# jrl-umi3218/jrl-walkgen

Measured on AMD Instinct MI355X. Metric: QP-MPC ticks/sec (batch=4096, N=16), higher is better.
Workload: dtype f64

## Files before the change

### jrl-walkgen_amd/csrc/wg_ql_device.hpp

```cpp
#pragma once
#include <hip/hip_runtime.h>

#include <type_traits>

#include "wg_wave.hpp"
#include "wg_ql_view.hpp"
#include "wg_ql_phases.hpp"

namespace wg {

#define WG_BACKSUB(q, s, nact, lane)                                                                   \
  do {                                                                                                 \
    if constexpr (P::kNM > 0 && P::kNM + 12 <= 48) backsub_lds<48>(q, s, nact, lane, q.sc0);          \
    else if (P::kNM == 0 && (P::kWideN || q.n >= 48) && (nact) <= 60) backsub_lds<96>(q, s, nact, lane, q.sc0);     \
    else if (P::kNM == 0 && !P::kRowOps && q.n >= 24 && (nact) <= 36) backsub_lds<48>(q, s, nact, lane, q.sc0); \
    else backsub(q, s, nact, lane);                                                                    \
  } while (0)
#define WG_SWEEP(q, s, nu, nact, lane) \
  do { if (P::kNM > 0 || (!P::kRowOps && q.n <= 64)) sweep_flat<P::kFixedLdz>(q, s, nu, nact, lane PT_SW_ARG); else sweep<(P::kRowOps ? WG_ELEM_GRP : 8), P::kWideN>(q, s, nu, nact, lane); } while (0)

#define QL_SCAN_ACCEPT                                                                        \
  if (wak <= 0.0) continue;                                                                   \
  double sumx = -sum * wak;                                                                   \
  if (k + 1 <= me) sumx = fabs(sumx);                                                         \
// ... 200 lines not shown
        xmag = 0.0;
        vfact = 1.0;
        WG_WSYNC();
        PT(PS_RESET_BODY);
      } else {
        iflag = 2;
        WG_REP(11) {
        typename ActiveParamsOf<P>::type ap;
        if constexpr (P::kCompact) ap = prob.active_params(q, nact, lane);
        for (int i = lane; i < n; i += 64) {
          double acc = q.d[i];
          if constexpr (P::kCompact) acc = prob.gdot_acc(q, i, q.x, acc);
          else {
            WG_UNROLL
            for (int j = 0; j < n; ++j) acc += Gm(i, j) * q.x[j];
          }
          PT_VIA(PS_RESID_GX, q.ww[i], acc);
          if constexpr (P::kCompact) acc = prob.grad_minus_active(q, ap, nact, i, acc);
          else {
            WG_UNROLL
            for (int k = 0; k < nact; ++k) {
              int kk = q.iact[k];
              if (kk <= m) acc -= q.lam[k] * Am(kk - 1, i);
              else if (kk <= mn) { if (kk - m - 1 == i) acc -= q.lam[k]; }
              else { if (kk - mn - 1 == i) acc += q.lam[k]; }
            }
          }
          q.ww[i] = acc;
        }
        if constexpr (P::kCompact) { prob.row_residuals(q, q.sc0, lane); WG_WSYNC(); }
        for (int k = lane; k < nact; k += 64) {
          int kk = q.iact[k];
          double sk;
          if (kk <= m) {
            if constexpr (P::kCompact) sk = q.sc0[kk - 1];
            else {
              sk = q.b[kk - 1];
              WG_UNROLL
              for (int i = 0; i < n; ++i) sk -= q.x[i] * Am(kk - 1, i);
            }
          } else if (kk <= mn) { int k1 = kk - m - 1; sk = prob.xl(q, k1) - q.x[k1]; }
          else { int k1 = kk - mn - 1; sk = -prob.xu(q, k1) + q.x[k1]; }
          s[k] = sk;
        }
        WG_WSYNC();
        }
        PT(PS_RESID_GRAD);
      }
      if (nact > 0) {
        {
          double sum0 = 0.0, sum1 = 0.0;
          const int i0 = lane, i1 = lane + 64;
          for (int j = 0; j < nact; ++j) {
            if (i0 == j) s[j] = (s[j] - sum0) / Rp(j, j);
            if (i1 == j) s[j] = (s[j] - sum1) / Rp(j, j);
            WG_WSYNC();
            double sj = s[j];
            if (i0 > j && i0 < nact) sum0 += Rp(j, i0) * sj;
            if (i1 > j && i1 < nact) sum1 += Rp(j, i1) * sj;
          }
        }
        PT(PS_RESID_FWD);
        if (P::kWideN || (P::kNM == 0 && n > 64 && n <= 128)) {
          double r0, r1;
          z_rows_times<(P::kRowOps ? WG_ELEM_GRP : 8)>(q, s, 0, nact, lane, r0, r1);
          q.x[lane] += r0; q.sc0[lane] = r0;
          if (lane + 64 < n) { q.x[lane + 64] += r1; q.sc0[lane + 64] = r1; }
        } else
        for (int i = lane; i < n; i += 64) {
          double sum = 0.0;
          WG_UNROLL
          for (int j = 0; j < nact; ++j) sum += s[j] * Zm(i, j);
          q.x[i] += sum;
          q.sc0[i] = sum;
        }
        WG_WSYNC();
        for (int j = lane; j < n; j += 64) {
          double acc = q.ww[j];
          if constexpr (P::kCompact) acc = prob.gdot_acc(q, j, q.sc0, acc);
          else {
            WG_UNROLL
            for (int i = 0; i < n; ++i) acc += q.sc0[i] * Gm(i, j);
          }
          q.ww[j] = acc;
        }
        WG_WSYNC();
      }
      PT(PS_RESID);
      zt_times_ww<P::kNM, (P::kRowOps ? WG_ELEM_GRP : 8), P::kWideN>(q, s, lane);
      PT(PS_ZTWW_RESID);
      if (nact != n) {
        if (P::kWideN || (P::kNM == 0 && n > 64 && n <= 128)) {
          double r0, r1;
          z_rows_times<(P::kRowOps ? WG_ELEM_GRP : 8)>(q, s, nact, n, lane, r0, r1);
          q.x[lane] -= r0;
          if (lane + 64 < n) q.x[lane + 64] -= r1;
        } else
        for (int i = lane; i < n; i += 64) {
          double sum = 0.0;
          WG_UNROLL
          for (int j = nact; j < n; ++j) sum += Zm(i, j) * s[j];
          q.x[i] -= sum;
        }
        info = 0;
        WG_WSYNC();
      }
      PT(PS_XSHIFT);
      if (nact != 0) {
        WG_BACKSUB(q, s, nact, lane);
        for (int k = lane; k < nact; k += 64) q.lam[k] += q.ww[k];
        WG_WSYNC();
      }
      PT(PS_BACKSUB_RESID);
      { double sm = 0.0; WG_REP(6) { sm = uni(xmag_sum(q, prob, vfact, lane)); WG_SINK(sm); } xmag = maxd(xmag, sm); }
      PT(PS_XMAG_RESID);
      if (iflag == itref) { st = ST_RESID; continue; }
      int kd = 0x7fffffff;
      for (int k = lane; k < nact; k += 64)
        if (!(q.lam[k] >= 0.0) && q.iact[k] > me) { kd = k < kd ? k : kd; }
      kd = uni(wave_min_int(kd));
      if (kd != 0x7fffffff) {
        LOG_EVENT(-q.iact[kd]);
        nact = drop_constraint(q, kd, nact, nact, lane);
        st = ST_RESID;
        continue;
      }
      if constexpr (kNan) x_suspect = x_suspect || x_has_non_numbers();
      st = ST_SCAN;
    }

    if (st == ST_SCAN) {
      next_scan: asm volatile("" : "+v"(lane));
      double bestv = 0.0, bestres = 0.0, bestw = 0.0;
      int bidx = -1;
      if (kNan && x_suspect) {
        if constexpr (kNan) {
          double cv = 0.0;
          int kn = knext;
          scan_nan_exact(q, prob, onha, cv, res, wsel, kn, lane);
          knext = uni(kn);
          bestv = uni(cv); bidx = -1;
        }
      } else
      WG_REP(1) {
      bestv = 0.0; bestres = 0.0; bestw = 0.0; bidx = -1;
      if constexpr (P::kCompact) {
        constexpr int NH = sizeof(prob.ax) / sizeof(double);
        double xs[2 * NH];
#pragma unroll
        for (int c = 0; c < 2 * NH; ++c) xs[c] = q.x[c];
        const bool has_foot = lane < 5 * prob.ns;
        const int kf = has_foot ? 1 + 4 * NH + lane : 0;
        const double wakf = q.wa[kf], bkf = q.b[kf];
        {
          const int k = lane + 1;
          const double wak = q.wa[k], bk = prob.bcop;
          double sum = -bk, asum = fabs(bk);
          prob.cop_row_dot(xs, sum, asum);
          if (prob.fj >= 0) {
            double t = q.x[2 * NH + prob.fj] * prob.fa(); sum += t; asum += fabs(t);
            t = q.x[2 * NH + prob.ns + prob.fj] * prob.fb(); sum += t; asum += fabs(t);
          }
          const double sumx = -sum * wak;
          {
            const double tempa = asum + fabs(sum);
            const double temp2 = asum + onha * fabs(sum);
            const bool take = (wak > 0.0) & !(sumx <= 0.0) & !(tempa <= asum) & !(temp2 <= tempa);
            bestv = take ? sumx : bestv; bestres = take ? sum : bestres; bestw = take ? wak : bestw; bidx = take ? k + 1 : bidx;
          }
        }
        {
          const int k = kf;
          const double wak = wakf, bk = bkf;
          double sum = -bk, asum = fabs(bk);
          const auto fr = prob.foot_row();
#pragma unroll
          for (int e = 0; e < 4; ++e) { const double t = q.x[fr.c[e]] * fr.v[e]; sum += t; asum += fabs(t); }
          const double sumx = -sum * wak;
          const double tempa = asum + fabs(sum);
          const double temp2 = asum + onha * fabs(sum);
          const bool take = has_foot & (wak > 0.0) & !(sumx <= 0.0) & !((bidx >= 0) & (sumx <= bestv)) & !(tempa <= asum) & !(temp2 <= tempa);
          bestv = take ? sumx : bestv; bestres = take ? sum : bestres; bestw = take ? wak : bestw; bidx = take ? k + 1 : bidx;
        }
      } else {
      if constexpr (P::kRowOps) {
        constexpr int kScanPasses = 3;
        double wak_p[kScanPasses], bk_p[kScanPasses], ra_p[kScanPasses], rb_p[kScanPasses];
        int rk_p[kScanPasses];
#pragma unroll
        for (int pp = 0; pp < kScanPasses; ++pp) {
          const int k = 1 + 64 * pp + lane;
          const bool in = k < m;
          const int kc = in ? k : 0;
          wak_p[pp] = in ? q.wa[kc] : 0.0; bk_p[pp] = q.b[kc];
          ra_p[pp] = prob.rowA[kc]; rb_p[pp] = prob.rowB[kc]; rk_p[pp] = prob.rowK[kc];
        }
#pragma unroll
        for (int pp = 0; pp < kScanPasses; ++pp) {
          const int k0 = 1 + 64 * pp;
          if (k0 >= m) break;
          const int k = k0 + lane;
          const int kc = k < m ? k : 0;
          const double wak = wak_p[pp], bk = bk_p[pp];
          double sum = -bk, temp = fabs(bk);
          prob.row_dot_both(q, kc, k0, ra_p[pp], rb_p[pp], rk_p[pp], q.x, sum, temp);
          QL_SCAN_ACCEPT;
        }
      } else if constexpr (HasRegRows<P>::value) {
        constexpr int NMr = P::kNM;
        const int ka = lane, kb = lane + 64;
        const bool ina = ka < m, inb = kb < m;
        const int mc = m > 0 ? m - 1 : 0;
        const int kca = ina ? ka : mc, kcb = inb ? kb : mc;
        const double waka = ina ? q.wa[kca] : 0.0, bka = q.b[kca], wakb = inb ? q.wa[kcb] : 0.0, bkb = q.b[kcb];
        double suma = -bka, tempa_ = fabs(bka), sumb = -bkb, tempb_ = fabs(bkb);
#pragma unroll
        for (int i0 = 0; i0 < NMr; i0 += 8) {
          double xs[8];
#pragma unroll
          for (int e = 0; e < 8; ++e) xs[e] = q.x[(i0 + e < n) ? i0 + e : n - 1];
#pragma unroll
          for (int e = 0; e < 8; ++e)
            if (i0 + e < NMr && i0 + e < n) {
              const double ta = xs[e] * prob.ar0[i0 + e]; suma += ta; tempa_ += fabs(ta);
              const double tb = xs[e] * prob.ar1[i0 + e]; sumb += tb; tempb_ += fabs(tb);
            }
        }
#pragma unroll
        for (int pp = 0; pp < 2; ++pp) {
          const int k = pp == 0 ? ka : kb;
          const double wak = pp == 0 ? waka : wakb, sum = pp == 0 ? suma : sumb;
          double temp = pp == 0 ? tempa_ : tempb_;
          QL_SCAN_ACCEPT;
        }
      } else
      for (int k0 = 0; k0 < m; k0 += 64) {
        const int k = k0 + lane;
        const bool in = k < m;
        const int kc = in ? k : m - 1;
        const double wak = in ? q.wa[kc] : 0.0, bk = q.b[kc];
        double sum = -bk, temp = fabs(bk);
        {
          constexpr int kG = 8;
          double ua[kG], ub[kG];
          auto fetch = [&](double (&u)[kG], int i) {
#pragma unroll
            for (int e = 0; e < kG; ++e) u[e] = Am(kc, i + e < n ? i + e : n - 1);
          };
          auto add = [&](const double (&u)[kG], int i) {
            double xs[kG];
#pragma unroll
            for (int e = 0; e < kG; ++e) xs[e] = q.x[i + e];
#pragma unroll
            for (int e = 0; e < kG; ++e) { const double t = xs[e] * u[e]; sum += t; temp += fabs(t); }
          };
          int i = 0;
          const int whole = n / kG * kG;
          if (whole > 0) {
            fetch(ua, 0);
            for (;;) {
              fetch(ub, i + kG);
              add(ua, i); i += kG;
              if (i >= whole) break;
              fetch(ua, i + kG);
              add(ub, i); i += kG;
              if (i >= whole) { 
#pragma unroll
                for (int e = 0; e < kG; ++e) ub[e] = ua[e];
                break;
              }
            }
#pragma unroll
            for (int e = 0; e < kG - 1; ++e)
              if (i + e < n) { const double t = q.x[i + e] * ub[e]; sum += t; temp += fabs(t); }
          } else {
            for (; i < n; ++i) { const double t = q.x[i] * Am(kc, i); sum += t; temp += fabs(t); }
          }
        }
        QL_SCAN_ACCEPT;
      }
      }
      if constexpr (P::kNM > 0) {
        const bool in = lane < n;
        const int kc = in ? lane : n - 1;
        const double w = q.wa[m + kc], xk = q.x[kc];
        const double s1 = prob.xl(q, kc) - xk;
        const bool upper = s1 < 0.0;
        const double sum = upper ? xk - prob.xu(q, kc) : s1;
        const bool take = in && !(w <= 0.0) && !(s1 == 0.0) && !(sum <= 0.0) && !(bidx >= 0 && sum <= bestv);
        bestv = take ? sum : bestv; bestres = take ? -sum : bestres; bestw = take ? w : bestw; bidx = take ? (upper ? kc + 1 + mn : kc + 1 + m) : bidx;
      } else
      for (int k = lane; k < n; k += 64) {
        const double w = q.wa[m + k];
        if (w <= 0.0) continue;
        bool lower = true;
        double sum = prob.xl(q, k) - q.x[k];
        if (sum == 0.0) continue;
        if (sum < 0.0) { sum = q.x[k] - prob.xu(q, k); lower = false; }
        if (sum <= 0.0) continue;
        if (bidx >= 0 && sum <= bestv) continue;
        bestv = sum; bestres = -sum; bestw = w; bidx = lower ? k + 1 + m : k + 1 + mn;
      }
      {
        int key = bidx < 0 ? -1 : (bidx > mn ? bidx - n : bidx);
        double v = bestv;
        int kk = key;
        wave_argmax_first(v, kk);
        kk = uni(kk);
        if (kk < 0) { bestv = 0.0; bidx = -1; }
        else {
          int src = -1;
          unsigned long long mask = __ballot(key == kk);
          src = __ffsll((long long)mask) - 1;
          bestv = rl(bestv, src);
          bestres = rl(bestres, src);
          bestw = rl(bestw, src);
          bidx = __builtin_amdgcn_readlane(bidx, src);
        }
      }
      WG_SINK(bestv); WG_SINK(bestres); WG_SINK(bestw); WG_SINK(bidx);
      }
      double cvmax = bestv;
      if (bidx >= 0) { res = bestres; knext = bidx; wsel = bestw; }
      PT(PS_SCAN);
      info = 0;
      if (WG_UBOOL(cvmax <= wg_kconst(vsmall))) { st = ST_CONVERGED; continue; }

      ++jfinc;
      if (jfinc == 0 || jfinc == ifinc) {
        if (jfinc == ifinc) {
          for (int i = lane; i < n; i += 64) {
            double sum = 2.0 * q.d[i];
            double sumx = fabs(sum);
            WG_UNROLL
            for (int j = 0; j < n; ++j) {
              double temp = Gm(i, j) * (q.wx[j] + q.x[j]);
              sum += temp;
              sumx += fabs(temp);
            }
            double dx = q.x[i] - q.wx[i];
            q.sc0[i] = sum * dx;
            q.sc1[i] = sumx * fabs(dx);
          }
          WG_WSYNC();
          double fdiff = 0.0, fdiffa = 0.0;
          WG_UNROLL
          for (int i = 0; i < n; ++i) { fdiff += q.sc0[i]; fdiffa += q.sc1[i]; }
          info = 2;
          double sum = fdiffa + fdiff;
          if (WG_UBOOL(sum <= fdiffa)) { st = ST_CONVERGED; continue; }
          double temp = fdiffa + onha * fdiff;
          if (WG_UBOOL(temp <= sum)) { st = ST_CONVERGED; continue; }
          jfinc = 0;
          info = 0;
        }
        for (int i = lane; i < n; i += 64) q.wx[i] = q.x[i];
        WG_WSYNC();
      }
      PT(PS_FDIFF);
      ++iterc;
      if (iterc > maxit) { info = 1; st = ST_FINISH; continue; }

      s = q.R + nact * (nact + 1) / 2;
      WG_REP(2)
      if (knext <= m) {
        if constexpr (P::kCompact) prob.fill_row(q, knext - 1, q.ww, lane);
        else if constexpr (HasRegRows<P>::value) prob.row_to(q, knext - 1, q.ww, lane);
        else for (int i = lane; i < n; i += 64) q.ww[i] = Am(knext - 1, i);
        WG_WSYNC();
        if constexpr (P::kCompact) prob.zt_row(q, s, knext - 1, lane);
        else if constexpr (P::kWideN && P::kRowOps) {
          constexpr int kNHc = P::kHorizon;
          const int k = knext - 1;
          const bool cop = k >= 1 && k <= 4 * kNHc;
          const int rr = cop ? ((k - 1) >> 2) : -1;
          const int si = cop ? prob.stepidx[rr] : 1;
          zt_times_ww_cop_tiled<kNHc>(q, s, lane, rr, !cop || (si >= 1 && si <= prob.ns));
        }
        else zt_times_ww<P::kNM, (P::kRowOps ? WG_ELEM_GRP : 8), P::kWideN>(q, s, lane);
      } else {
        int k1 = knext - m;
        double sg = 1.0;
        if (k1 > n) { k1 = knext - mn; sg = -1.0; }
        for (int i = lane; i < n; i += 64) {
          q.ww[i] = (i == k1 - 1) ? sg : 0.0;
          double z = Zm(k1 - 1, i);
          s[i] = (sg > 0.0) ? z : -z;
        }
        WG_WSYNC();
      }
      PT(PS_NEWNORMAL);
      double parnew = 0.0, parinc = 0.0, step = 0.0, sumy;
      int kdrop = -1;
      int route;
      if (nact == n) route = 1;
      else {
        WG_SWEEP(q, s, n, nact, lane);
        PT(PS_SWEEP);
        if (nact == 0) route = 0;
        else {
          double suma = 0.0, sumb = 0.0, sumc = 0.0;
          WG_REP(5) {
          if constexpr (P::kNM > 0) {
            constexpr int NM = P::kNM;
            if (lane < NM) {
              const bool in = lane < n;
              const double zi = in ? Zm(lane, nact) : 0.0, wi = in ? q.ww[lane] : 0.0;
              q.sc0[lane] = wi * zi; q.sc1[lane] = fabs(wi * zi); q.sc2[lane] = zi * zi;
            }
            WG_WSYNC();
            typedef __attribute__((address_space(3))) double lds_f64;
            const lds_f64 *src = (const lds_f64 *)(q.sc0 + (lane < 3 ? lane : 0) * (int)(q.sc1 - q.sc0));
            asm volatile("" : "+v"(src));
            double acc = 0.0;
#pragma unroll
            for (int i0 = 0; i0 < NM; i0 += kOsChunk) {
              double t[kOsChunk];
#pragma unroll
              for (int i = 0; i < kOsChunk; ++i) if (i0 + i < NM) t[i] = src[i0 + i];
#pragma unroll
              for (int i = 0; i < kOsChunk; ++i) if (i0 + i < NM) acc += t[i];
            }
            suma = rl(acc, 0); sumb = rl(acc, 1); sumc = rl(acc, 2);
            WG_WSYNC();
          } else {
            for (int i = lane; i < n; i += 64) {
              const double zi = Zm(i, nact), wi = q.ww[i];
              q.sc0[i] = wi * zi; q.sc1[i] = fabs(wi * zi); q.sc2[i] = zi * zi;
            }
            WG_WSYNC();
            const double *src = q.sc0 + (lane < 3 ? lane : 0) * (int)(q.sc1 - q.sc0);
            double acc = 0.0;
            int i = 0;
            for (; i + 8 <= n; i += 8) {
              double t[8];
#pragma unroll
              for (int e = 0; e < 8; ++e) t[e] = src[i + e];
#pragma unroll
              for (int e = 0; e < 8; ++e) acc += t[e];
            }
            for (; i < n; ++i) acc += src[i];
            suma = rl(acc, 0); sumb = rl(acc, 1); sumc = rl(acc, 2);
            WG_WSYNC();
          }
          WG_SINK(suma); WG_SINK(sumb); WG_SINK(sumc);
          }
          if (WG_UBOOL(!significant(sumb, fabs(suma)) || !(sumb > wg_kconst(vsmall)))) route = 1;
          else {
            sumc = sqrt(sumc);
            if (knext <= m) sumc /= wsel;
            if (WG_UBOOL(significant(sumc, fabs(suma)))) route = 0;
            else {
              PT_COUNT(PS_N_COORD);
              WG_BACKSUB(q, s, nact, lane);
              route = independent_coordinate(q, prob, knext, nact, vsmall, lane) ? 0 : 2;
            }
          }
        }
      }
      route = uni(route);
      PT(PS_ROUTE);
      PT_COUNT(PS_N_ROUTE);
      if (route != 0) PT_COUNT(PS_N_DEPENDENT);
      if (route != 0) {
        if (route == 1) WG_BACKSUB(q, s, nact, lane);
        kdrop = pick_drop<(P::kNM > 0), kNan>(q, nact, res, ratio, lane);
        info = -knext;
        if (kdrop < 0) { st = ST_CONVERGED; continue; }
        parinc = ratio;
        parnew = parinc;
      }

      bool dual_only = (route != 0);
      for (;;) {
        if (!dual_only) {
          sumy = s[nact];
          step = -res / sumy;
          parinc = step / sumy;
          kdrop = -1;
          if (nact > 0) {
            PT(PS_STEP_PRE);
            WG_REP(4) WG_BACKSUB(q, s, nact, lane);
            PT(PS_BACKSUB_STEP);
            WG_REP(7) { kdrop = pick_drop<(P::kNM > 0), kNan>(q, nact, res, ratio, lane); WG_SINK(kdrop); WG_SINK(ratio); }
            PT(PS_PICKDROP);
            if (kdrop >= 0) {
              double temp = 1.0 - ratio / parinc;
              if (WG_UBOOL(temp <= 0.0)) kdrop = -1;
              else { step = ratio * sumy; parinc = ratio; res = temp * res; }
            }
          }
          if constexpr (P::kNM > 0) {
            const int il = lane < n ? lane : n - 1;
            q.x[il] = q.x[il] + step * Zm(il, nact);
          } else
          for (int i = lane; i < n; i += 64) q.x[i] += step * Zm(i, nact);
          parnew += parinc;
          if constexpr (kNan) x_suspect = x_suspect || WG_UBOOL(!wg_sane(step) || !wg_sane(parinc));
          WG_WSYNC();
          if (nact < 1) break;
        }
        dual_only = false;
        if constexpr (P::kNM > 0) {
          if (nact > 0) {
            const int kl = lane < nact ? lane : nact - 1;
            const double l0 = q.lam[kl] - parinc * q.ww[kl];
            const int ia = q.iact[kl];
            q.lam[kl] = (ia > me) ? maxd(0.0, l0) : l0;
          }
        } else
        for (int k = lane; k < nact; k += 64) {
          double l = q.lam[k] - parinc * q.ww[k];
          if (q.iact[k] > me) l = maxd(0.0, l);
          q.lam[k] = l;
        }
        WG_WSYNC();
        if (kdrop < 0) break;
        {
          int nu = nact + 1;
          LOG_EVENT(-q.iact[kdrop]);
          nact = drop_constraint(q, kdrop, nu, nact, lane);
          double *snew = s - (nact + 1);
          if (nu > n) nu = n;
          for (int i0 = 0; i0 < nu; i0 += 64) {
            int i = i0 + lane;
            double v = (i < nu) ? s[i] : 0.0;
            WG_WSYNC();
            if (i < nu) snew[i] = v;
            WG_WSYNC();
          }
          s = snew;
          WG_SWEEP(q, s, nu, nact, lane);
        }
      }

      PT(PS_STEP);
      ql_activate(q, nact, knext, parnew, wsel, lane, n, mn);
      nact++;
      LOG_EVENT(knext);
      WG_WSYNC();
      PT(PS_ADD);
      double sm = 0.0;
      WG_REP(6) { sm = uni(xmag_sum(q, prob, vfact, lane)); WG_SINK(sm); }
      xmag = maxd(xmag, sm);
      PT(PS_XMAG_ADD);
      if (WG_UBOOL(sm < wg_kconst(xmagr) * xmag)) st = ST_RESET;
      else if (itref <= 0) st = ST_SCAN;
      else st = ST_RESID;
      if (q.nact_cap > 0 && nact > q.nact_cap) { cap_hit = true; break; }
      if (st == ST_SCAN) goto next_scan;
      continue;
    }

    if (st == ST_CONVERGED) {
      ++itref;
      jfinc = -1;
      if (itref == 1) { st = ST_RESID; continue; }
      st = ST_FINISH;
    }
  }
#undef LOG_EVENT
// ... 20 lines not shown
```

### jrl-walkgen_amd/csrc/wg_ql_herdt.hpp

```cpp
#pragma once
#include "wg_ql_device.hpp"

namespace wg {

constexpr int kSMaxQ = 4;
constexpr int kGvLd = 4;
constexpr int kQbLd = 32;

template <int NH, int NS>
__device__ __forceinline__ bool herdt_border_rows(const QlView &q, const double *gd, const double *Gv, double vsmall, int lane) {
  constexpr int M2 = 2 * NH;
  const int i = lane;
  const bool jerk = i < NH, foot = i >= NH && i < NH + NS, row = jerk || foot;
  const int fi = i - NH;
  const int gi = jerk ? i : M2 + (foot ? fi : 0);
  double acc[NS];
#pragma unroll
  for (int f = 0; f < NS; ++f)
    acc[f] = (jerk || (foot && f >= fi)) ? ((foot && f == fi) ? gd[gi] : Gv[gi * kGvLd + f]) : 0.0;
  const double dreg = jerk ? Rf(i, i) : 1.0;
  const int colbase = jerk ? i * (i + 1) / 2 : 0;
  const int khi = jerk ? i : 0;
  double rnext = (0 < khi) ? q.Rf[colbase] : 0.0;
  for (int k = 0; k < NH; ++k) {
// ... 363 lines not shown
    }
    const int cc = row - 2 * NH;
#pragma unroll
    for (int k0 = 0; k0 < 2 * NH; k0 += 8) {
      double gg[8], vv[8];
#pragma unroll
      for (int c = 0; c < 8; ++c) { gg[c] = Gv[(k0 + c) * kGvLd + cc]; vv[c] = v[k0 + c]; }
#pragma unroll
      for (int c = 0; c < 8; ++c) acc += gg[c] * vv[c];
    }
    for (int c = 0; c < n - 2 * NH; ++c) {
      const double g = (c == cc) ? gd[row] : Gv[row * kGvLd + c];
      acc += g * v[2 * NH + c];
    }
    return acc;
  }

  struct ActiveParams { double pa, pb, plam; int pr, ptype, pidx; };
  __device__ __forceinline__ ActiveParams active_params(const QlView &q, int nact, int lane) const {
    const int m = q.m, mn = q.mn;
    ActiveParams P;
    P.pa = 0.0; P.pb = 0.0; P.plam = 0.0; P.pr = -1; P.ptype = 4; P.pidx = -1;
    int rk = 0;
    if (lane < nact) {
      const int kk = q.iact[lane];
      P.plam = q.lam[lane];
      if (kk <= m) {
        rk = kk - 1;
        P.ptype = (rk >= 1 && rk <= 4 * NH) ? 0 : 1;
        if (rk == 0) P.ptype = 4;
      } else if (kk <= mn) { P.ptype = 2; P.pidx = kk - m - 1; }
      else { P.ptype = 3; P.pidx = kk - mn - 1; }
    }
    double *t = q.sc0;
    t[lane + 1] = ra;
    if (lane < 5 * ns) t[1 + 4 * NH + lane] = ga;
    WG_WSYNC();
    if (P.ptype <= 1) P.pa = t[rk];
    WG_WSYNC();
    t[lane + 1] = rb;
    if (lane < 5 * ns) t[1 + 4 * NH + lane] = gb;
    WG_WSYNC();
    if (P.ptype <= 1) P.pb = t[rk];
    WG_WSYNC();
    int *tk = reinterpret_cast<int *>(q.sc0);
    if (lane < 5 * ns) tk[lane] = gk;
    WG_WSYNC();
    if (P.ptype == 0) P.pr = (rk - 1) >> 2;
    else if (P.ptype == 1) P.pr = tk[rk - 1 - 4 * NH];
    WG_WSYNC();
    return P;
  }
  __device__ __forceinline__ double grad_minus_active(const QlView &q, const ActiveParams &P, int nact, int i, double acc) const {
    const bool xb = i < NH, jerk = i < 2 * NH;
    const int c = xb ? i : i - NH;
    int fjx = -1, fjy = -1;
    if (!jerk) { const int j = i - 2 * NH; if (j < ns) fjx = j; else fjy = j - ns; }
    for (int k = 0; k < nact; ++k) {
      const int type = __builtin_amdgcn_readlane(P.ptype, k);
      const double lam = rl(P.plam, k);
      if (type <= 1) {
        const double a = rl(P.pa, k), b = rl(P.pb, k);
        const int r = __builtin_amdgcn_readlane(P.pr, k);
        double e = 0.0;
        if (type == 0) {
          if (jerk) {
            const double ab = xb ? a : b;
            const int rc = (c <= r) ? r - c : 0;
            const double uu = u[rc];
            e = (c <= r) ? 0.0 + (0.0 + ab * uu) * -1.0 : 0.0;
          } else {
            const int sidx = stepidx[r];
            if (fjx >= 0) { const double v = (sidx == fjx + 1) ? 1.0 : 0.0; e = 0.0 + (0.0 + a * v) * 1.0; }
            else { const double v = (sidx == fjy + 1) ? 1.0 : 0.0; e = 0.0 + (0.0 + b * v) * 1.0; }
          }
        } else if (!jerk && r >= 0) {
          if (fjx >= 0) e = 0.0 + (0.0 + a * V_f[r * kSMaxQ + fjx]) * -1.0;
          else e = 0.0 + (0.0 + b * V_f[r * kSMaxQ + fjy]) * -1.0;
        }
        acc -= lam * e;
      } else if (type == 2) {
        if (__builtin_amdgcn_readlane(P.pidx, k) == i) acc -= lam;
      } else if (type == 3) {
        if (__builtin_amdgcn_readlane(P.pidx, k) == i) acc += lam;
      }
    }
    return acc;
  }
  __device__ __forceinline__ void row_residuals(const QlView &q, double *out, int lane) const {
    double xs[2 * NH];
#pragma unroll
    for (int c = 0; c < 2 * NH; ++c) xs[c] = q.x[c];
    {
      const int rk = lane + 1;
      double sk = q.b[rk];
#pragma unroll
      for (int c = 0; c < NH; ++c) sk -= xs[c] * ax[c];
#pragma unroll
      for (int c = 0; c < NH; ++c) sk -= xs[NH + c] * ay[c];
      if (fj >= 0) { sk -= q.x[2 * NH + fj] * fa(); sk -= q.x[2 * NH + ns + fj] * fb(); }
      out[rk] = sk;
    }
    if (lane < 5 * ns) {
      const int rk = 1 + 4 * NH + lane;
      double sk = q.b[rk];
      const FootRow fr = foot_row();
#pragma unroll
      for (int e = 0; e < 4; ++e) sk -= q.x[fr.c[e]] * fr.v[e];
      out[rk] = sk;
    }
    if (lane == 0) out[0] = q.b[0];
  }

  __device__ __forceinline__ double diag_check(const QlView &q, double vsmall, int lane) const {
    const int n = q.n;
    double dl = diag_b;
    for (int i = lane; i < n; i += 64) {
      const double wdi = q.wd[i];
      if (i >= 2 * NH) dl = maxd(dl, vsmall - wdi);
      const int j0 = (i + 1 > 2 * NH) ? i + 1 : 2 * NH;
      for (int j = j0; j < n; ++j) {
        const double gjj = q.wd[j], gij = G(q, i, j);
        double ga = -mind(wdi, gjj);
        const double gb = fabs(wdi - gjj) + fabs(gij);
        if (gb > 0.0) ga += gij * gij / gb;
        dl = maxd(dl, ga);
      }
    }
    return wave_max(dl);
  }

  __device__ __forceinline__ bool factor(const QlView &q, double vsmall, int lane) const {
    const int n = q.n;
    constexpr int M2 = 2 * NH;
    PT_LOCAL_BEGIN
    herdt_constant_blocks<NH>(q, R2, Z2, z2sign, lane);
    WG_WSYNC();
    const int nb = n - M2;
    PT_LOCAL(PS_CHOL);
    bool ok = true;
    if (nb == 2) ok = herdt_border_rows<NH, 1>(q, gd, Gv, vsmall, lane);
    else if (nb == 4) ok = herdt_border_rows<NH, 2>(q, gd, Gv, vsmall, lane);
    if (!WG_UBOOL(ok)) return false;
    WG_WSYNC();
    PT_LOCAL(PS_BORDER_ROWS);
    if (nb == 2) herdt_border_z<NH, 1>(q, lane);
    else if (nb == 4) herdt_border_z<NH, 2>(q, lane);
    WG_WSYNC();
    return true;
  }

  __device__ __forceinline__ void zt_row(const QlView &q, double *s, int rk, int lane) const {
    const int n = q.n;
    if (lane < n) {
      const int i = lane;
      const double *zc = q.Z + i * q.ldz;
      double acc = 0.0;
      if (rk >= 1 && rk <= 4 * NH) {
        constexpr int kZtChunk = 8;
        const int r = (rk - 1) >> 2;
#pragma unroll
        for (int j0 = 0; j0 < 2 * NH; j0 += kZtChunk) {
          if ((j0 < NH ? j0 : j0 - NH) > r) continue;
          double zz[kZtChunk], wv[kZtChunk];
#pragma unroll
          for (int c = 0; c < kZtChunk; ++c) { zz[c] = zc[j0 + c]; wv[c] = q.ww[j0 + c]; }
#pragma unroll
          for (int c = 0; c < kZtChunk; ++c) acc += zz[c] * wv[c];
        }
      }
      for (int j = 2 * NH; j < n; ++j) acc += zc[j] * q.ww[j];
      s[i] = acc;
    }
    WG_WSYNC();
  }
};

constexpr int kGvLdElem = kSMaxQ;
template <int NHC>
struct HerdtElemProbT {
  static constexpr bool kCompact = false;
  static constexpr bool kNanExact = WG_TICK_NAN_EXACT != 0;
  static constexpr bool kHasFactor = true;
  static constexpr bool kRowOps = true;
  static constexpr int kNM = 0;
  static constexpr bool kWideN = NHC >= 32;
  static constexpr int kFixedLdz = 0;
  static constexpr int kHorizon = NHC;
  struct NConst { static constexpr int v = NHC; __device__ __forceinline__ NConst &operator=(int) { return *this; } __device__ __forceinline__ operator int() const { return v; } };
  typename std::conditional<(NHC > 0), NConst, int>::type N;
  int ns;
  const double *Qb;
  const double *u;
  double *Gv;
  double *gd;
  const double *rowA, *rowB;
  const int *rowK, *stepidx;
  const double *V_f;
  const double *R2, *Z2;
  const unsigned long long *z2sign;
  int blocks_ok;
  __device__ __forceinline__ bool factor(const QlView &q, double vsmall, int lane) const {
    if ((int)N != 32 || ns < 1 || ns > 4) return false;
    constexpr int NHc = 32;
    herdt_constant_blocks<NHc>(q, R2, Z2, z2sign, lane);
    WG_WSYNC();
    bool ok = true;
    switch (ns) {
      case 1: ok = herdt_border_rows<NHc, 1>(q, gd, Gv, vsmall, lane); break;
      case 2: ok = herdt_border_rows<NHc, 2>(q, gd, Gv, vsmall, lane); break;
      case 3: ok = herdt_border_rows<NHc, 3>(q, gd, Gv, vsmall, lane); break;
      default: ok = herdt_border_rows<NHc, 4>(q, gd, Gv, vsmall, lane); break;
    }
    if (!WG_UBOOL(ok)) return false;
    WG_WSYNC();
    switch (ns) {
      case 1: herdt_border_z<NHc, 1>(q, lane); break;
      case 2: herdt_border_z<NHc, 2>(q, lane); break;
      case 3: herdt_border_z<NHc, 3>(q, lane); break;
      default: herdt_border_z<NHc, 4>(q, lane); break;
    }
    WG_WSYNC();
    return true;
  }
  __device__ __forceinline__ double G(const QlView &q, int i, int j) const {
    if (i == j) return gd[i];
    if (j < i) { const int t = i; i = j; j = t; }
    if (j < 2 * N) {
      if (i < N && j < N) return Qb[i * kQbLd + j];
      if (i >= N && j >= N) return Qb[(i - N) * kQbLd + (j - N)];
      return 0.0;
    }
    const int c = j - 2 * N;
    const bool xcol = c < ns, xrow = (i < N) || (i >= 2 * N && i < 2 * N + ns);
    if (xcol != xrow) return 0.0;
    return Gv[i * kGvLdElem + (xcol ? c : c - ns)];
  }
  __device__ __forceinline__ double Gd(const QlView &, int i) const { return gd[i]; }
  __device__ __forceinline__ void setGd(const QlView &, int i, double v) const { gd[i] = v; }
  __device__ __forceinline__ double xl(const QlView &, int) const { return -1e8; }
  __device__ __forceinline__ double xu(const QlView &, int) const { return 1e8; }
  __device__ __forceinline__ double A(const QlView &, int k, int i) const {
    if (k == 0) return 0.0;
    const double a = rowA[k], b = rowB[k];
    const int kk = rowK[k];
    if (k <= 4 * N) {
      const int r = kk;
      if (i < N) return (i <= r) ? 0.0 + (0.0 + a * u[r - i]) * -1.0 : 0.0;
      if (i < 2 * N) { const int c = i - N; return (c <= r) ? 0.0 + (0.0 + b * u[r - c]) * -1.0 : 0.0; }
      int j = i - 2 * N;
      if (j < ns) { const double v = (stepidx[r] == j + 1) ? 1.0 : 0.0; return 0.0 + (0.0 + a * v) * 1.0; }
      j -= ns;
      { const double v = (stepidx[r] == j + 1) ? 1.0 : 0.0; return 0.0 + (0.0 + b * v) * 1.0; }
    }
    if (kk < 0 || i < 2 * N) return 0.0;
    int j = i - 2 * N;
    if (j < ns) return 0.0 + (0.0 + a * V_f[kk * kSMaxQ + j]) * -1.0;
    j -= ns;
    return 0.0 + (0.0 + b * V_f[kk * kSMaxQ + j]) * -1.0;
  }
  template <bool ABS>
  __device__ __forceinline__ double row_dot(const QlView &, int k, const double *v, double acc) const {
    if (k == 0) return acc;
    const double a = rowA[k], b = rowB[k];
    const int kk = rowK[k];
    if (k <= 4 * N) {
      const int r = kk;
      for (int c = 0; c <= r; ++c) { const double t = v[c] * (0.0 + (0.0 + a * u[r - c]) * -1.0); acc += ABS ? fabs(t) : t; }
      for (int c = 0; c <= r; ++c) { const double t = v[N + c] * (0.0 + (0.0 + b * u[r - c]) * -1.0); acc += ABS ? fabs(t) : t; }
      const int j = stepidx[r] - 1;
      if (j >= 0 && j < ns) {
        { const double t = v[2 * N + j] * (0.0 + (0.0 + a * 1.0) * 1.0); acc += ABS ? fabs(t) : t; }
        { const double t = v[2 * N + ns + j] * (0.0 + (0.0 + b * 1.0) * 1.0); acc += ABS ? fabs(t) : t; }
      }
      return acc;
    }
    if (kk < 0) return acc;
    for (int j = 0; j < ns; ++j) { const double t = v[2 * N + j] * (0.0 + (0.0 + a * V_f[kk * kSMaxQ + j]) * -1.0); acc += ABS ? fabs(t) : t; }
    for (int j = 0; j < ns; ++j) { const double t = v[2 * N + ns + j] * (0.0 + (0.0 + b * V_f[kk * kSMaxQ + j]) * -1.0); acc += ABS ? fabs(t) : t; }
    return acc;
  }
  __device__ __forceinline__ void row_dot_both(const QlView &q, int k, int k0, const double *v, double &sum, double &asum) const {
    row_dot_both(q, k, k0, rowA[k], rowB[k], rowK[k], v, sum, asum);
  }
  __device__ __forceinline__ void row_dot_both(const QlView &, int k, int k0, double a, double b, int kk, const double *v, double &sum,
                                               double &asum) const {
    if (k0 <= 4 * N) {
      const bool cop = k >= 1 && k <= 4 * N;
      const int r = cop ? kk : -1;
      const int klast = (k0 + 63 < 4 * N) ? k0 + 63 : 4 * N;
      const int rmax = (klast - 1) >> 2;
      const double ac = cop ? a : 0.0, bc = cop ? b : 0.0;
#ifndef WG_SCAN_CH
#define WG_SCAN_CH 4
#endif
      constexpr int CH = WG_SCAN_CH;
#pragma unroll 1
      for (int c0 = 0; c0 <= rmax; c0 += CH) {
        double vv[CH], uu[CH];
#pragma unroll
        for (int e = 0; e < CH; ++e) { const int d = r - c0 - e, ci = c0 + e < N ? c0 + e : N - 1; vv[e] = v[ci]; uu[e] = u[d > -1 ? d : -1]; }
#pragma unroll
        for (int e = 0; e < CH; ++e) { const double t = vv[e] * (0.0 - ac * uu[e]); sum += t; asum += fabs(t); }
      }
#pragma unroll 1
      for (int c0 = 0; c0 <= rmax; c0 += CH) {
        double vv[CH], uu[CH];
#pragma unroll
        for (int e = 0; e < CH; ++e) { const int d = r - c0 - e, ci = c0 + e < N ? c0 + e : N - 1; vv[e] = v[N + ci]; uu[e] = u[d > -1 ? d : -1]; }
#pragma unroll
        for (int e = 0; e < CH; ++e) { const double t = vv[e] * (0.0 - bc * uu[e]); sum += t; asum += fabs(t); }
      }
      const int j = (r >= 0) ? stepidx[r] - 1 : -1;
      const bool st = j >= 0 && j < ns;
      const int jc = st ? j : 0;
      { const double t = v[2 * N + jc] * ((st ? a : 0.0) * 1.0 + 0.0); sum += t; asum += fabs(t); }
      { const double t = v[2 * N + ns + jc] * ((st ? b : 0.0) * 1.0 + 0.0); sum += t; asum += fabs(t); }
    }
    if (k0 + 63 > 4 * N) {
      const bool ft = k > 4 * N && kk >= 0;
      const int kf = ft ? kk : 0;
      const double af = ft ? a : 0.0, bf = ft ? b : 0.0;
      for (int j = 0; j < ns; ++j) { const double t = v[2 * N + j] * (0.0 - af * V_f[kf * kSMaxQ + j]); sum += t; asum += fabs(t); }
      for (int j = 0; j < ns; ++j) { const double t = v[2 * N + ns + j] * (0.0 - bf * V_f[kf * kSMaxQ + j]); sum += t; asum += fabs(t); }
// ... 28 lines not shown
```

### jrl-walkgen_amd/csrc/wg_ql_phases.hpp

```cpp
#pragma once
#include <hip/hip_runtime.h>

#include <type_traits>

#include "wg_wave.hpp"
#include "wg_ql_view.hpp"

namespace wg {

#ifndef WG_ELEM_GRP
#define WG_ELEM_GRP 4
#endif

__device__ __forceinline__ double sqrt_1to2(double x) {
  const double y = __builtin_amdgcn_rsq(x);
  double g = x * y;
  double h = y * 0.5;
  const double r = __builtin_fma(-h, g, 0.5);
  g = __builtin_fma(g, r, g);
  h = __builtin_fma(h, r, h);
  double d = __builtin_fma(-g, g, x);
  g = __builtin_fma(d, h, g);
  d = __builtin_fma(-g, g, x);
  g = __builtin_fma(d, h, g);
// ... 528 lines not shown
        constexpr int L = kLdzC;
        lds_f64 *zb = (lds_f64 *)(q.Z + i + nact * L);
        const lds_f64 *gb_ = (const lds_f64 *)(gab + 2 * nact);
        asm volatile("" : "+v"(zb), "+v"(gb_));
        auto rot = [&](const Op &o, int k) {
          const double t = o.ga * o.zl + o.gb * carry;
          zb[k * L] = o.ga * carry - o.gb * o.zl;
          carry = t;
        };
        auto ld = [&](int k) -> Op { Op o; o.zl = zb[(k - 1) * L]; o.ga = gb_[2 * k]; o.gb = gb_[2 * k + 1]; return o; };
        switch (c - nact) {
          case 5: { const Op o2 = ld(2), o1 = ld(1); rot(s0, 5); rot(s1, 4); rot(s2, 3); rot(o2, 2); rot(o1, 1); break; }
          case 4: { const Op o1 = ld(1); rot(s0, 4); rot(s1, 3); rot(s2, 2); rot(o1, 1); break; }
          case 3: rot(s0, 3); rot(s1, 2); rot(s2, 1); break;
          case 2: rot(s0, 2); rot(s1, 1); break;
          default: rot(s0, 1); break;
        }
        zb[0] = carry;
      } else {
      for (;;) {
        { const Op nx = fetch(c - 3); rotate_all(s0); s0 = nx; }
        if (--c <= nact) break;
        { const Op nx = fetch(c - 3); rotate_all(s1); s1 = nx; }
        if (--c <= nact) break;
        { const Op nx = fetch(c - 3); rotate_all(s2); s2 = nx; }
        if (--c <= nact) break;
      }
      zp[0] = carry;
      }
    }
    if (any_skip) zp[0] = carry;
  }
  WG_WSYNC();
  PT_SW(PS_SW_ROWS);
}

#ifndef WG_TICK_NAN_EXACT
#define WG_TICK_NAN_EXACT 1
#endif
#ifndef WG_NAN_REGIME
#define WG_NAN_REGIME 1
#endif
__device__ __forceinline__ bool wg_sane(double v) { return ((unsigned)__double2hiint(v) & 0x7fffffffu) < 0x54b00000u; }

template <class P>
__device__ __forceinline__ void scan_nan_exact(const QlView &q, const P &prob, double onha, double &cvmax, double &res,
                                               double &wsel, int &knext, int lane) {
  const int n = q.n, m = q.m, me = q.me, mn = q.mn;
  struct Row { bool cand; double v, r, w; int code; };
  auto eval = [&](int pos) -> Row {
    Row o;
    if (pos < m) {
      const int k = pos;
      o.w = q.wa[k];
      const double bk = q.b[k];
      double sum = -bk, temp = fabs(bk);
      for (int i = 0; i < n; ++i) {
        double aki;
        if constexpr (P::kCompact) aki = prob.A_own(k, i); else aki = Am(k, i);
        const double t = q.x[i] * aki; sum += t; temp += fabs(t);
      }
      o.v = -sum * o.w;
      if (k + 1 <= me) o.v = fabs(o.v);
      const double tempa = temp + fabs(sum);
      const double temp2 = temp + onha * fabs(sum);
      o.cand = !(o.w <= 0.0) && !(tempa <= temp) && !(temp2 <= tempa);
      o.r = sum; o.code = k + 1;
    } else {
      const int k = pos - m;
      o.w = q.wa[m + k];
      const double xk = q.x[k], s1 = prob.xl(q, k) - xk;
      const bool upper = s1 < 0.0;
      o.v = upper ? xk - prob.xu(q, k) : s1;
      o.cand = !(o.w <= 0.0) && !(s1 == 0.0);
      o.r = -o.v; o.code = upper ? k + 1 + mn : k + 1 + m;
    }
    return o;
  };
  auto position = [&](int j) -> int {
    if constexpr (P::kCompact) {
      if (j == 0) return (lane + 1 <= P::kCopRows && lane + 1 < m) ? lane + 1 : -1;
      if (j == 1) return (1 + P::kCopRows + lane < m) ? 1 + P::kCopRows + lane : -1;
      return lane < n ? m + lane : -1;
    } else {
      const int pos = lane + 64 * j;
      return pos < m + n ? pos : -1;
    }
  };
  const int slots = P::kCompact ? 3 : (m + n + 63) / 64;
  double av = 0.0, ar = 0.0, aw = 0.0;
  int apos = -1, acode = 0;
  double nr = 0.0, nw = 0.0;
  int npos = -1, ncode = 0;
  for (int j = 0; j < slots; ++j) {
    const int pos = position(j);
    if (pos < 0) continue;
    const Row o = eval(pos);
    if (!o.cand) continue;
    if (o.v != o.v) { npos = pos; nr = o.r; nw = o.w; ncode = o.code; }
    else if (o.v > av) { av = o.v; ar = o.r; aw = o.w; apos = pos; acode = o.code; }
  }
  const int lastnan = uni(wave_max_int(npos));
  int src;
  if (lastnan >= 0) {
    bool any = false;
    av = 0.0; apos = -1;
    for (int j = 0; j < slots; ++j) {
      const int pos = position(j);
      if (pos <= lastnan) continue;
      const Row o = eval(pos);
      if (!o.cand) continue;
      if (!any || o.v > av) { av = o.v; ar = o.r; aw = o.w; apos = pos; acode = o.code; }
      any = true;
    }
    if (__ballot(any) == 0ull) {
      src = __ffsll((long long)__ballot(npos == lastnan)) - 1;
      cvmax = __builtin_nan(""); res = rl(nr, src); wsel = rl(nw, src); knext = __builtin_amdgcn_readlane(ncode, src);
      return;
    }
  }
  double v = av;
  int kk = apos;
  wave_argmax_first(v, kk);
  kk = uni(kk);
  cvmax = 0.0;
  if (kk < 0) return;
  src = __ffsll((long long)__ballot(apos == kk)) - 1;
  cvmax = rl(av, src); res = rl(ar, src); wsel = rl(aw, src); knext = __builtin_amdgcn_readlane(acode, src);
}

__device__ __forceinline__ int pick_drop_serial_reference(const QlView &q, int nact, double res, double &ratio) {
  int kdrop = -1;
  for (int k = 0; k < nact; ++k) {
    if (q.iact[k] <= q.me) continue;
    const double w = q.ww[k];
    if (res * w >= 0.0) continue;
    const double temp = q.lam[k] / w;
    if (kdrop >= 0 && fabs(temp) >= fabs(ratio)) continue;
    kdrop = k; ratio = temp;
  }
  return kdrop;
}

__device__ __forceinline__ unsigned wave_min_u32(unsigned v) {
  asm("s_nop 1\n\tv_min_u32_dpp %0, %0, %0 row_shr:1 row_mask:0xf bank_mask:0xf\n\t"
      "s_nop 1\n\tv_min_u32_dpp %0, %0, %0 row_shr:2 row_mask:0xf bank_mask:0xf\n\t"
      "s_nop 1\n\tv_min_u32_dpp %0, %0, %0 row_shr:4 row_mask:0xf bank_mask:0xf\n\t"
      "s_nop 1\n\tv_min_u32_dpp %0, %0, %0 row_shr:8 row_mask:0xf bank_mask:0xf\n\t"
      "s_nop 1\n\tv_min_u32_dpp %0, %0, %0 row_bcast:15 row_mask:0xf bank_mask:0xf\n\t"
      "s_nop 1\n\tv_min_u32_dpp %0, %0, %0 row_bcast:31 row_mask:0xf bank_mask:0xf"
      : "+v"(v));
  return (unsigned)__builtin_amdgcn_readlane((int)v, 63);
}

template <bool kOnePass = false, bool kNan = false>
__device__ __forceinline__ int pick_drop(const QlView &q, int nact, double res, double &ratio, int lane) {
  double best = 0.0, bestt = 0.0;
  int bidx = -1;
  bool bad = !wg_sane(res);
  if constexpr (kOnePass) {
    const bool in = lane < nact;
    const int kc = in ? lane : 0;
    const double w = q.ww[kc];
    const int ia = q.iact[kc];
    const bool cand = in & (ia > q.me) & !(res * w >= 0.0);
    const double lamv = q.lam[kc];
    const double temp = lamv / w;
    if constexpr (kNan) {
      const bool bw = !wg_sane(w), bl = !wg_sane(lamv);
      bad = bad || (in && (bw || bl));
      if (__ballot(bad) != 0ull) return uni(pick_drop_serial_reference(q, nact, res, ratio));
      const unsigned hi = cand ? ((unsigned)__double2hiint(temp) & 0x7fffffffu) : 0xffffffffu;
      const unsigned lo = (unsigned)__double2loint(temp);
      const unsigned mh = wave_min_u32(hi);
      const unsigned ml = wave_min_u32(hi == mh ? lo : 0xffffffffu);
      const unsigned long long win = __ballot(cand && hi == mh && lo == ml);
      if (win == 0ull) return -1;
      const int idx = __ffsll((long long)win) - 1;
      ratio = rl(temp, idx);
      return idx;
    }
    best = cand ? -fabs(temp) : 0.0; bestt = cand ? temp : 0.0; bidx = cand ? lane : -1;
  } else
  for (int k = lane; k < nact; k += 64) {
    const double w = q.ww[k], lamv = q.lam[k];
    if constexpr (kNan) {
      const bool bw = !wg_sane(w), bl = !wg_sane(lamv);
      bad = bad || bw || bl;
    }
    if (q.iact[k] <= q.me) continue;
    if (res * w >= 0.0) continue;
    double temp = lamv / w;
    double key = -fabs(temp);
    if (bidx < 0 || key > best) { best = key; bestt = temp; bidx = k; }
  }
  if constexpr (kNan)
    if (__ballot(bad) != 0ull) return uni(pick_drop_serial_reference(q, nact, res, ratio));
  int idx = bidx;
  double v = best;
  wave_argmax_first(v, idx);
  idx = uni(idx);
  if (idx < 0) return -1;
  ratio = rl(bestt, idx & 63);
  return idx;
}

template <class P>
__device__ __forceinline__ double xmag_sum(const QlView &q, const P &prob, double vfact, int lane) {
  const int n = q.n;
  if constexpr (P::kNM > 0) {
    const int il = lane < n ? lane : n - 1;
    const double xi = q.x[il];
    const double term = fabs(xi) * vfact * (fabs(q.d[il]) + fabs(prob.Gd(q, il) * xi));
    return ordered_sum_lds<P::kNM>(term, q.sc3, n, lane);
  }
  for (int i = lane; i < n; i += 64) {
    double xi = q.x[i];
    q.sc3[i] = fabs(xi) * vfact * (fabs(q.d[i]) + fabs(prob.Gd(q, i) * xi));
  }
  WG_WSYNC();
  double sum = 0.0;
  int i = 0;
  for (; i + 8 <= n; i += 8) {
    double t[8];
#pragma unroll
    for (int e = 0; e < 8; ++e) t[e] = q.sc3[i + e];
#pragma unroll
    for (int e = 0; e < 8; ++e) sum += t[e];
  }
  for (; i < n; ++i) sum += q.sc3[i];
  return sum;
}

template <int GRP = 8, bool kWide = false>
__device__ __forceinline__ void sweep(const QlView &q, double *s, int nu, int nact, int lane) {
  const int n = q.n;
  if (nu - 1 <= nact) return;
  if (!kWide && n <= 64) {
    const double sreg = (lane < nu) ? s[lane] : 0.0;
    double myP = 0.0, myQ = 0.0, myN = 0.0;
    {
      double cur = rl(sreg, nu - 1);
      for (int c = nu - 1; c > nact; --c) {
        const double p = rl(sreg, c - 1);
        double nrm;
        if (cur == 0.0) { nrm = 0.0; cur = p; }
        else { nrm = givens_norm(p, cur); if (lane == c) { myP = p; myQ = cur; } cur = nrm; }
        if (lane == c) myN = nrm;
      }
    }
    double ga = 1.0, gb = 0.0;
    if (lane > nact && lane < nu && myN != 0.0) {
      ga = myP / myN;
      gb = myQ / myN;
      s[lane - 1] = myN;
    }
    {
      const int i = lane;
      const bool act = i < n;
      double carry = act ? Zm(i, nu - 1) : 0.0;
      double zl = act ? Zm(i, nu - 2) : 0.0;
      for (int c = nu - 1; c > nact; --c) {
        const double zn = (act && c - 2 >= nact) ? Zm(i, c - 2) : 0.0;
        const double nc = rl(myN, c);
        if (nc == 0.0) { if (act) Zm(i, c) = carry; carry = zl; }
        else {
          const double gac = rl(ga, c), gbc = rl(gb, c);
          const double t = gac * zl + gbc * carry;
          if (act) Zm(i, c) = gac * carry - gbc * zl;
          carry = t;
        }
        zl = zn;
      }
      if (act) Zm(i, nact) = carry;
    }
    WG_WSYNC();
    return;
  }
  double *chain = q.sc3;
  WG_REP(3)
  if (sweep_range_ok(s, nact, nu, lane)) {
    double cur = s[nu - 1];
    double pa = s[nu - 2], pb;
    int c = nu - 1;
    int iv = nu - 4;
    asm volatile("" : "+v"(iv));
    const int rots = c - nact;
    if (WG_UBOOL(cur != 0.0)) {
      for (int k = rots >> 1; k > 0; --k) {
        pb = s[iv + 1];
        cur = givens_norm_fast(pa, cur); chain[iv + 2] = cur;
        pa = s[iv];
        cur = givens_norm_fast(pb, cur); chain[iv + 1] = cur;
        iv -= 2;
      }
      if (rots & 1) { cur = givens_norm_fast(pa, cur); chain[iv + 2] = cur; }
    } else {
      for (int k = rots >> 1; k > 0; --k) {
        pb = s[iv + 1];
        { const double nrmc = givens_norm_fast(pa, cur); cur = (cur == 0.0) ? pa : nrmc; chain[iv + 2] = cur; }
        pa = s[iv];
        { const double nrmc = givens_norm_fast(pb, cur); cur = (cur == 0.0) ? pb : nrmc; chain[iv + 1] = cur; }
        iv -= 2;
      }
      if (rots & 1) { const double nrmc = givens_norm_fast(pa, cur); cur = (cur == 0.0) ? pa : nrmc; chain[iv + 2] = cur; }
    }
// ... 271 lines not shown
```

Before: 6.679 million.

## Fuse bound scan into compact scan and use integer-DPP argmax lane selection

For the compact problem, the solver now hoists the x loads for the step and foot rows and folds the variable-bound violation check into the same branch-free constraint scan, skipping the separate bound loop. The winning lane is picked by a new integer DPP max reduction on the high and low words of the positive double, with ties broken by minimum key, replacing the generic wave argmax. Divergent lane guards in the Z^T row product and the NM scratch fill are replaced by clamped indices, and the Z^T tail is fully unrolled for at most four entries. This reduces divergence and reduction latency, at the cost of redundant duplicate work on inactive lanes and reliance on positive-double bit ordering.

After: 6.817 million (median of 6 runs). 1.02x the previous value.

```diff
diff --git a/jrl-walkgen_amd/csrc/wg_ql_device.hpp b/jrl-walkgen_amd/csrc/wg_ql_device.hpp
--- a/jrl-walkgen_amd/csrc/wg_ql_device.hpp
+++ b/jrl-walkgen_amd/csrc/wg_ql_device.hpp
@@ -376,14 +376,24 @@
         const bool has_foot = lane < 5 * prob.ns;
         const int kf = has_foot ? 1 + 4 * NH + lane : 0;
         const double wakf = q.wa[kf], bkf = q.b[kf];
+        const bool has_step = prob.fj >= 0;
+        const double xsa = q.x[has_step ? 2 * NH + prob.fj : 0], xsb = q.x[has_step ? 2 * NH + prob.ns + prob.fj : 0];
+        const auto fr = prob.foot_row();
+        double xfr[4];
+#pragma unroll
+        for (int e = 0; e < 4; ++e) xfr[e] = q.x[fr.c[e]];
+        const bool bin = lane < n;
+        const int bkc = bin ? lane : n - 1;
+        const double bw = q.wa[m + bkc], bxk = q.x[bkc];
         {
           const int k = lane + 1;
           const double wak = q.wa[k], bk = prob.bcop;
           double sum = -bk, asum = fabs(bk);
           prob.cop_row_dot(xs, sum, asum);
-          if (prob.fj >= 0) {
-            double t = q.x[2 * NH + prob.fj] * prob.fa(); sum += t; asum += fabs(t);
-            t = q.x[2 * NH + prob.ns + prob.fj] * prob.fb(); sum += t; asum += fabs(t);
+          {
+            const double ca = has_step ? prob.fa() : 0.0, cb = has_step ? prob.fb() : 0.0;
+            double t = xsa * ca; sum += t; asum += fabs(t);
+            t = xsb * cb; sum += t; asum += fabs(t);
           }
           const double sumx = -sum * wak;
           {
@@ -397,14 +407,21 @@
           const int k = kf;
           const double wak = wakf, bk = bkf;
           double sum = -bk, asum = fabs(bk);
-          const auto fr = prob.foot_row();
-#pragma unroll
-          for (int e = 0; e < 4; ++e) { const double t = q.x[fr.c[e]] * fr.v[e]; sum += t; asum += fabs(t); }
+#pragma unroll
+          for (int e = 0; e < 4; ++e) { const double t = xfr[e] * fr.v[e]; sum += t; asum += fabs(t); }
           const double sumx = -sum * wak;
           const double tempa = asum + fabs(sum);
           const double temp2 = asum + onha * fabs(sum);
           const bool take = has_foot & (wak > 0.0) & !(sumx <= 0.0) & !((bidx >= 0) & (sumx <= bestv)) & !(tempa <= asum) & !(temp2 <= tempa);
           bestv = take ? sumx : bestv; bestres = take ? sum : bestres; bestw = take ? wak : bestw; bidx = take ? k + 1 : bidx;
+        }
+        {
+          const double s1 = prob.xl(q, bkc) - bxk;
+          const bool upper = s1 < 0.0;
+          const double sum = upper ? bxk - prob.xu(q, bkc) : s1;
+          const bool take = bin & !(bw <= 0.0) & !(s1 == 0.0) & !(sum <= 0.0) & !((bidx >= 0) & (sum <= bestv));
+          bestv = take ? sum : bestv; bestres = take ? -sum : bestres; bestw = take ? bw : bestw;
+          bidx = take ? bkc + 1 + m + (upper ? n : 0) : bidx;
         }
       } else {
       if constexpr (P::kRowOps) {
@@ -504,7 +521,8 @@
         QL_SCAN_ACCEPT;
       }
       }
-      if constexpr (P::kNM > 0) {
+      if constexpr (P::kCompact) {
+      } else if constexpr (P::kNM > 0) {
         const bool in = lane < n;
         const int kc = in ? lane : n - 1;
         const double w = q.wa[m + kc], xk = q.x[kc];
@@ -527,6 +545,16 @@
       }
       {
         int key = bidx < 0 ? -1 : (bidx > mn ? bidx - n : bidx);
+        if constexpr (P::kCompact) {
+          const int src = scan_select_lane(bestv, key);
+          if (src < 0) { bestv = 0.0; bidx = -1; }
+          else {
+            bestv = rl(bestv, src);
+            bestres = rl(bestres, src);
+            bestw = rl(bestw, src);
+            bidx = __builtin_amdgcn_readlane(bidx, src);
+          }
+        } else {
         double v = bestv;
         int kk = key;
         wave_argmax_first(v, kk);
@@ -540,6 +568,7 @@
           bestres = rl(bestres, src);
           bestw = rl(bestw, src);
           bidx = __builtin_amdgcn_readlane(bidx, src);
+        }
         }
       }
       WG_SINK(bestv); WG_SINK(bestres); WG_SINK(bestw); WG_SINK(bidx);
@@ -627,10 +656,13 @@
           WG_REP(5) {
           if constexpr (P::kNM > 0) {
             constexpr int NM = P::kNM;
-            if (lane < NM) {
-              const bool in = lane < n;
-              const double zi = in ? Zm(lane, nact) : 0.0, wi = in ? q.ww[lane] : 0.0;
-              q.sc0[lane] = wi * zi; q.sc1[lane] = fabs(wi * zi); q.sc2[lane] = zi * zi;
+            {
+              const int il = lane < NM ? lane : NM - 1;
+              const bool in = il < n;
+              const int ic = in ? il : n - 1;
+              const double zv = Zm(ic, nact), wv = q.ww[ic];
+              const double zi = in ? zv : 0.0, wi = in ? wv : 0.0;
+              q.sc0[il] = wi * zi; q.sc1[il] = fabs(wi * zi); q.sc2[il] = zi * zi;
             }
             WG_WSYNC();
             typedef __attribute__((address_space(3))) double lds_f64;
diff --git a/jrl-walkgen_amd/csrc/wg_ql_herdt.hpp b/jrl-walkgen_amd/csrc/wg_ql_herdt.hpp
--- a/jrl-walkgen_amd/csrc/wg_ql_herdt.hpp
+++ b/jrl-walkgen_amd/csrc/wg_ql_herdt.hpp
@@ -539,8 +539,8 @@
 
   __device__ __forceinline__ void zt_row(const QlView &q, double *s, int rk, int lane) const {
     const int n = q.n;
-    if (lane < n) {
-      const int i = lane;
+    {
+      const int i = lane < n ? lane : n - 1;
       const double *zc = q.Z + i * q.ldz;
       double acc = 0.0;
       if (rk >= 1 && rk <= 4 * NH) {
@@ -556,7 +556,14 @@
           for (int c = 0; c < kZtChunk; ++c) acc += zz[c] * wv[c];
         }
       }
-      for (int j = 2 * NH; j < n; ++j) acc += zc[j] * q.ww[j];
+      constexpr int kTail = kNM - 2 * NH;
+      static_assert(kTail == 4, "two entries per previewed step, at most two steps");
+      double zt[kTail], wt[kTail];
+#pragma unroll
+      for (int c = 0; c < kTail; ++c) { zt[c] = zc[2 * NH + c]; wt[c] = q.ww[2 * NH + c]; }
+      const int nb = n - 2 * NH;
+      if (nb >= 2) { acc += zt[0] * wt[0]; acc += zt[1] * wt[1]; }
+      if (nb >= 4) { acc += zt[2] * wt[2]; acc += zt[3] * wt[3]; }
       s[i] = acc;
     }
     WG_WSYNC();
diff --git a/jrl-walkgen_amd/csrc/wg_ql_phases.hpp b/jrl-walkgen_amd/csrc/wg_ql_phases.hpp
--- a/jrl-walkgen_amd/csrc/wg_ql_phases.hpp
+++ b/jrl-walkgen_amd/csrc/wg_ql_phases.hpp
@@ -704,6 +704,34 @@
       : "+v"(v));
   return (unsigned)__builtin_amdgcn_readlane((int)v, 63);
 }
+__device__ __forceinline__ unsigned wave_max_u32(unsigned v) {
+  asm("s_nop 1\n\tv_max_u32_dpp %0, %0, %0 row_shr:1 row_mask:0xf bank_mask:0xf\n\t"
+      "s_nop 1\n\tv_max_u32_dpp %0, %0, %0 row_shr:2 row_mask:0xf bank_mask:0xf\n\t"
+      "s_nop 1\n\tv_max_u32_dpp %0, %0, %0 row_shr:4 row_mask:0xf bank_mask:0xf\n\t"
+      "s_nop 1\n\tv_max_u32_dpp %0, %0, %0 row_shr:8 row_mask:0xf bank_mask:0xf\n\t"
+      "s_nop 1\n\tv_max_u32_dpp %0, %0, %0 row_bcast:15 row_mask:0xf bank_mask:0xf\n\t"
+      "s_nop 1\n\tv_max_u32_dpp %0, %0, %0 row_bcast:31 row_mask:0xf bank_mask:0xf"
+      : "+v"(v));
+  return (unsigned)__builtin_amdgcn_readlane((int)v, 63);
+}
+
+__device__ __forceinline__ int scan_select_lane(double v, int key) {
+  const bool cand = key >= 0 && v > 0.0;
+  const unsigned hi = cand ? (unsigned)__double2hiint(v) : 0u;
+  const unsigned mh = wave_max_u32(hi);
+  const bool top = cand && hi == mh;
+  const unsigned lo = top ? (unsigned)__double2loint(v) : 0u;
+  const unsigned ml = wave_max_u32(lo);
+  const bool winl = top && lo == ml;
+  const unsigned long long win = __ballot(winl);
+  if (win == 0ull) return -1;
+  int src = __ffsll((long long)win) - 1;
+  if ((win & (win - 1ull)) != 0ull) {
+    const unsigned kmin = wave_min_u32(winl ? (unsigned)key : 0xffffffffu);
+    src = __ffsll((long long)__ballot(winl && (unsigned)key == kmin)) - 1;
+  }
+  return src;
+}
 
 template <bool kOnePass = false, bool kNan = false>
 __device__ __forceinline__ int pick_drop(const QlView &q, int nact, double res, double &ratio, int lane) {
```
